# mlvlab/BLiM

Measured on AMD Instinct MI355X. Metric: candidate-pairs/sec (7B, 96+32 tok), higher is better.
Workload: dtype f16; 1 GPU; SYN v2t-VTG re-rank: Qwen2-7B dims (28 layers), seeded synthetic weights, 96 video + 32 text tokens per pair, top-16 text candidates per video query, 55 queries (880 pairs, 32560 packed tokens, 28160 label rows) per step per GPU; prefix_reuse=True, vtg_compensated=none, parallelism=query rows sharded over 1 GPU(s); RCCL all-gather of score rows at the end

## Files before the change

### blim_amd/csrc/gemm.hip

```cpp
#include "gemm.hpp"
#include "kernels.hpp"
#include <type_traits>

#define BM 256
#define BN 256
#define BK 64
#define NTHREADS 512
#define TILE_BYTES (BM * BK * 2)
#define BUF_BYTES (2 * TILE_BYTES)
#define GROUP_M 8

typedef const __attribute__((address_space(1))) void* gptr_t;
typedef __attribute__((address_space(3))) void* lptr_t;

__device__ __forceinline__ void glds16(const void* g, char* lds_wave_base) {
    __builtin_amdgcn_global_load_lds((gptr_t)g, (lptr_t)lds_wave_base, 16, 0, 0);
}

__device__ __forceinline__ float gelu_erf(float x) {
    const float z = fabsf(x) * 0.70710678118654752f;
    const float t = __builtin_amdgcn_rcpf(fmaf(0.3275911f, z, 1.0f));
    const float poly = t * fmaf(t, fmaf(t, fmaf(t, fmaf(t, 1.061405429f, -1.453152027f), 1.421413741f), -0.284496736f), 0.254829592f);
    const float erf_abs = 1.0f - poly * __expf(-z * z);
    return 0.5f * x * (1.0f + copysignf(erf_abs, x));
// ... 189 lines not shown
                    }
                    dma1(q);
                }
#ifdef GEMM_ABLATE_WREAD
#pragma unroll
                for (int ks = 0; ks < 2; ++ks)
#pragma unroll
                    for (int r = 0; r < 4; ++r) fb[ks][r] = fa[ks][r + 4];
#endif
            }
        };
        typedef int i32x2 __attribute__((ext_vector_type(2)));
        const char* g6A = LO6 ? (const char*)p.A6 + (int64_t)tm * nk6 * F6_TILE_BYTES : nullptr;
        const char* g6W = LO6 ? (const char*)p.W6 + (int64_t)tn * nk6 * F6_TILE_BYTES : nullptr;
        uint2 sc6a = make_uint2(0, 0);
        uint32_t sc6w = 0;
        auto dma6 = [&](int q, int dslot, int kd, bool isW, bool on) __attribute__((always_inline)) {
#if defined(GEMM_ABLATE_P2) && GEMM_ABLATE_P2 == 3
            on = on && kd < 3;
#endif
#if defined(GEMM_ABLATE_P2) && GEMM_ABLATE_P2 >= 4
            on = on && !((q == 4 || q == 5) && (isW || GEMM_ABLATE_P2 == 5));
#endif
            if (on) {
                const char* g = (isW ? g6W : g6A) + (int64_t)kd * F6_TILE_BYTES;
                char* d = smem + dslot * F6_TILE_BYTES;
                uint32_t o16 = (uint32_t)lane * 16u;
                asm volatile("" : "+v"(o16));
                if (q < 6) glds16(g + (wg + 4 * q) * 1024 + o16, d + (wg + 4 * q) * 1024);
                else if (lane < 16) glds16(g + 24576 + wg * 256 + o16, d + 24576 + wg * 256);
            }
        };
        auto stage6 = [&](int slot, int k, bool isW) __attribute__((always_inline)) {
#pragma unroll
            for (int q = 0; q < 7; ++q) dma6(q, slot, k, isW, true);
        };
        auto rd6 = [&](const char* qa, const char* qb, int off) __attribute__((always_inline)) {
            const i32x4 l = *(const i32x4*)(qa + off);
            const i32x2 h = *(const i32x2*)(qb + off);
            return (i32x8){l[0], l[1], l[2], l[3], h[0], h[1], 0, 0};
        };
#if defined(GEMM_ABLATE_P2) && GEMM_ABLATE_P2 >= 4
        auto rd6_4 = [&](const char* qa, const char* qb, int off) __attribute__((always_inline)) {
            const i32x4 l = *(const i32x4*)(qa + off);
            return (i32x8){l[0], l[1], l[2], l[3], l[0], l[1], 0, 0};
        };
#define RD6W rd6_4
#if GEMM_ABLATE_P2 == 5
#define RD6A rd6_4
#else
#define RD6A rd6
#endif
#else
#define RD6W rd6
#define RD6A rd6
#endif
        typedef int i32x1 __attribute__((ext_vector_type(1)));
        auto rd6_sw = [&](const char* tb) __attribute__((always_inline)) {
            return (uint32_t)(*(const i32x1*)(tb + 24576 + wn * 256 + lane * 4))[0];
        };
        auto rd6_sa = [&](const char* ta) __attribute__((always_inline)) {
            const i32x2 v = *(const i32x2*)(ta + 24576 + wm * 512 + lane * 8);
            return make_uint2((uint32_t)v[0], (uint32_t)v[1]);
        };
        int sa = 0;
        mx_request(0);
        if (grp == 0) {
            stage8(TILE_BYTES, 0);
            if (nk > 1) stage8(3 * TILE_BYTES, 1);
            if (nk > 1) asm volatile("s_waitcnt vmcnt(8)" ::: "memory");
            else asm volatile("s_waitcnt vmcnt(0)" ::: "memory");
            PHASE_BARRIER();
            if constexpr (MX8) mx_cur = mx_nxt;
            if constexpr (DT == DT_F8) {
                int sp = 0;
                for (int k = 0; k < nk; ++k) {
                    mx_request(k + 1);
                    load_frags(sa, adv(sa, 1));
                    if (k >= 1 && k + 1 < nk) stage8(sp, k + 1);
                    PHASE_BARRIER();
                    compute();
                    asm volatile("s_waitcnt vmcnt(0)" ::: "memory");
                    if constexpr (MX8) mx_cur = mx_nxt;
                    PHASE_BARRIER();
                    sp = sa; sa = adv(sa, 2);
                }
                PHASE_BARRIER();
            } else {
            load_frags(0, TILE_BYTES);
            PHASE_BARRIER();
            for (int kt = 0; kt < nk; ++kt) {
                WP_T(0);
                compute();
                WP_T(1);
                asm volatile("s_waitcnt vmcnt(0)" ::: "memory");
                WP_T(2);
                PHASE_BARRIER();
                WP_T(3);
                if constexpr (LO6) { if (kt + 1 == nk) break; }
                if (kt + 1 < nk) frags_and_dma(adv(sa, 2), adv(sa, 3), sa, kt + 2, kt + 2 < nk);
#ifdef GEMM_WAIT_PROF
                asm volatile("s_waitcnt lgkmcnt(0)" ::: "memory");
#endif
                WP_T(4);
                PHASE_BARRIER();
                WP_T(5);
                WP_ACC();
                sa = adv(sa, 2);
            }
            if constexpr (LO6) {
                stage6(0, 0, false); stage6(1, 0, true);
                if (nk6 > 1) { stage6(2, 1, false); stage6(3, 1, true); }
                if (nk6 > 2) { stage6(4, 2, false); stage6(5, 2, true); }
                PHASE_BARRIER();
            }
            }
        } else {
            stage8(0, 0);
            if (nk > 1) stage8(2 * TILE_BYTES, 1);
            if (nk > 1) asm volatile("s_waitcnt vmcnt(8)" ::: "memory");
            else asm volatile("s_waitcnt vmcnt(0)" ::: "memory");
            PHASE_BARRIER();
            if constexpr (MX8) mx_cur = mx_nxt;
            PHASE_BARRIER();
            for (int kt = 0; kt < nk; ++kt) {
                WP_T(0);
                if constexpr (DT == DT_F8) {
                    mx_request(kt + 1);
                    load_frags(sa, adv(sa, 1));
                    if (kt + 2 < nk) stage8(adv(sa, 4), kt + 2);
                } else frags_and_dma(sa, adv(sa, 1), adv(sa, 4), kt + 2, kt + 2 < nk);
#ifdef GEMM_WAIT_PROF
                asm volatile("s_waitcnt lgkmcnt(0)" ::: "memory");
#endif
                WP_T(1);
                if (kt + 2 < nk) asm volatile("s_waitcnt vmcnt(8)" ::: "memory");
                else asm volatile("s_waitcnt vmcnt(0)" ::: "memory");
                WP_T(2);
                PHASE_BARRIER();
                WP_T(3);
                compute();
                if constexpr (MX8) mx_cur = mx_nxt;
                WP_T(4);
                PHASE_BARRIER();
                WP_T(5);
                WP_ACC();
                sa = adv(sa, 2);
            }
        }
        if constexpr (LO6) {
#define P2_VMCNT(n) asm volatile("s_waitcnt vmcnt(" #n ")" ::: "memory")
#define P2_BARRIER() PHASE_BARRIER()
            if (grp == 0) {
                if (nk6 > 2) P2_VMCNT(28);
                else if (nk6 > 1) P2_VMCNT(14);
                else P2_VMCNT(0);
            }
            P2_BARRIER();
            const int qoa = 8 * wm * 1536 + lane * 16, qoa8 = 8 * wm * 1536 + 1024 + lane * 8;
            const int qob = F6_TILE_BYTES + 4 * wn * 1536 + lane * 16, qob8 = F6_TILE_BYTES + 4 * wn * 1536 + 1024 + lane * 8;
            sc6w = rd6_sw(smem + F6_TILE_BYTES); sc6a = rd6_sa(smem);
            fb8[0] = RD6W(smem + qob, smem + qob8, 0); fb8[1] = RD6W(smem + qob, smem + qob8, 1536);
#pragma unroll
            for (int i = 0; i < 4; ++i) fa8[i] = RD6A(smem + qoa, smem + qoa8, i * 1536);
            int s3 = 0;
#ifdef GEMM_WAIT_PROF
            for (int q_ = 0; q_ < 5; ++q_) wp_acc[q_] = 0;
#endif
#if defined(GEMM_ABLATE_P2) && GEMM_ABLATE_P2 == 1
#define L6_MMA(MI, NI)
#else
#define L6_MMA(MI, NI) acc[MI][NI] = __builtin_amdgcn_mfma_scale_f32_16x16x128_f8f6f4(fb8[NI], fa8[MI], acc[MI][NI], 2, 2, NI, (int)sc6w, (MI & 3), (int)((MI) < 4 ? sc6a.x : sc6a.y));
#endif
#define L6_SB() __builtin_amdgcn_sched_barrier(0)
            auto step6 = [&](int k, auto ca_, auto cb_) __attribute__((always_inline)) {
                constexpr int CA = decltype(ca_)::value, CB = decltype(cb_)::value;
                const int s3n = s3 == 2 ? 0 : s3 + 1, s3p = s3 == 0 ? 2 : s3 - 1;
                const char* t0 = smem + (2 * s3) * F6_TILE_BYTES;
                const char* t1 = smem + (2 * s3n) * F6_TILE_BYTES;
#if defined(GEMM_ABLATE_P2) && GEMM_ABLATE_P2 == 2
                const bool rl = false, own = false;
#else
                const bool rl = k + 1 < nk6, own = true;
#endif
                const bool on2 = k >= 1 && k + 2 < nk6;
                const bool on3 = k + 3 < nk6;
                const int d2 = 2 * s3p + (grp == 0 ? 1 : 0), d3 = 2 * s3 + (grp == 0 ? 1 : 0);
                const bool isW = grp == 0;
                uint2 sc6a_n = sc6a; uint32_t sc6w_n = sc6w;
                WP_T(0);
                __builtin_amdgcn_s_setprio(1);
                L6_MMA(0, CA) L6_SB(); if (own) fb8[CB] = RD6W(t0 + qob, t0 + qob8, CB * 1536); L6_SB();
                L6_MMA(1, CA) L6_SB(); dma6(4, d2, k + 2, isW, on2); L6_SB();
                L6_MMA(2, CA) L6_SB(); if (own) fb8[CB + 1] = RD6W(t0 + qob, t0 + qob8, (CB + 1) * 1536); L6_SB();
                L6_MMA(3, CA) L6_SB();
                L6_MMA(0, CA + 1) L6_SB(); if (own) fa8[4] = RD6A(t0 + qoa, t0 + qoa8, 4 * 1536); L6_SB();
                L6_MMA(1, CA + 1) L6_SB(); dma6(5, d2, k + 2, isW, on2); L6_SB();
                L6_MMA(2, CA + 1) L6_SB(); if (own) fa8[5] = RD6A(t0 + qoa, t0 + qoa8, 5 * 1536); L6_SB();
                L6_MMA(3, CA + 1) L6_SB();
                L6_MMA(0, CB) L6_SB(); if (own) fa8[6] = RD6A(t0 + qoa, t0 + qoa8, 6 * 1536); L6_SB();
                L6_MMA(1, CB) L6_SB(); if (own) fa8[7] = RD6A(t0 + qoa, t0 + qoa8, 7 * 1536); L6_SB();
                L6_MMA(2, CB) L6_SB(); dma6(6, d2, k + 2, isW, on2); L6_SB();
                L6_MMA(3, CB)
                L6_MMA(0, CB + 1) L6_MMA(1, CB + 1) L6_MMA(2, CB + 1) L6_MMA(3, CB + 1)
                L6_SB();
                WP_T(1);
#if defined(GEMM_ABLATE_P2) && GEMM_ABLATE_P2 == 6
                if (k == 0) { if (nk6 > 2) P2_VMCNT(21); else P2_VMCNT(0); }
                else if (k + 2 < nk6) P2_VMCNT(14);
                else P2_VMCNT(0);
#else
                if (k == 0) { if (nk6 > 2) P2_VMCNT(14); else P2_VMCNT(0); }
                else if (k + 2 < nk6) P2_VMCNT(7);
                else P2_VMCNT(0);
#endif
                WP_T(2);
#if defined(GEMM_ABLATE_P2) && GEMM_ABLATE_P2 == 7
                if (k & 1) { asm volatile("s_waitcnt lgkmcnt(0)" ::: "memory"); } else { P2_BARRIER(); }
#else
                P2_BARRIER();
#endif
                WP_T(3);
                L6_MMA(4, CB) L6_SB(); if (rl) fa8[0] = RD6A(t1 + qoa, t1 + qoa8, 0); L6_SB();
                L6_MMA(5, CB) L6_SB(); dma6(0, d3, k + 3, isW, on3); L6_SB();
                L6_MMA(6, CB) L6_SB(); if (rl) fa8[1] = RD6A(t1 + qoa, t1 + qoa8, 1536); L6_SB();
                L6_MMA(7, CB) L6_SB(); dma6(1, d3, k + 3, isW, on3); L6_SB();
                L6_MMA(4, CB + 1) L6_SB(); if (rl) { sc6w_n = rd6_sw(t1 + F6_TILE_BYTES); sc6a_n = rd6_sa(t1); } L6_SB();
                L6_MMA(5, CB + 1) L6_MMA(6, CB + 1) L6_MMA(7, CB + 1)
                L6_SB();
                WP_T(4);
                if (rl) fb8[CB] = RD6W(t1 + qob, t1 + qob8, CB * 1536);
                L6_SB();
                L6_MMA(4, CA) L6_SB(); if (rl) fb8[CB + 1] = RD6W(t1 + qob, t1 + qob8, (CB + 1) * 1536); L6_SB();
                L6_MMA(5, CA) L6_SB(); dma6(2, d3, k + 3, isW, on3); L6_SB();
                L6_MMA(6, CA) L6_SB(); if (rl) fa8[2] = RD6A(t1 + qoa, t1 + qoa8, 2 * 1536); L6_SB();
                L6_MMA(7, CA) L6_SB(); dma6(3, d3, k + 3, isW, on3); L6_SB();
                L6_MMA(4, CA + 1) L6_SB(); if (rl) fa8[3] = RD6A(t1 + qoa, t1 + qoa8, 3 * 1536); L6_SB();
                L6_MMA(5, CA + 1) L6_MMA(6, CA + 1) L6_MMA(7, CA + 1)
                L6_SB();
                __builtin_amdgcn_s_setprio(0);
                sc6a = sc6a_n; sc6w = sc6w_n;
                WP_T(5);
                WP_ACC();
                s3 = s3n;
            };
            {
                int k = 0;
                for (; k + 1 < nk6; k += 2) {
                    step6(k, std::integral_constant<int, 0>{}, std::integral_constant<int, 2>{});
                    step6(k + 1, std::integral_constant<int, 2>{}, std::integral_constant<int, 0>{});
                }
                if (k < nk6) step6(k, std::integral_constant<int, 0>{}, std::integral_constant<int, 2>{});
            }
#undef L6_SB
#undef RD6W
#undef RD6A
#undef P2_BARRIER
#undef P2_VMCNT
#undef L6_MMA
        }
#undef PHASE_BARRIER
#ifdef GEMM_WAIT_PROF
        if (p.debug_stamps && lane == 0 && (wave & 3) == 0)
            for (int q_ = 0; q_ < 5; ++q_) p.debug_stamps[((size_t)nwg + (size_t)stamp_vb * 2 + grp) * 8 + q_] = wp_acc[q_];
#endif
    }

    stamp(2);
    int tid_e = tid;
    asm volatile("" : "+v"(tid_e));
    if constexpr (out16<DT>::value == DT_F16) { if (p.f16_saturate) f16_saturate_on(); }
    else if constexpr (LO6_BF16_FENCE) { if (p.f16_saturate) f16_saturate_off(); }
    if (p.debug_skip_epilogue) {
#pragma unroll
        for (int i = 0; i < 8; ++i)
#pragma unroll
            for (int j = 0; j < 4; ++j) asm volatile("" ::"v"(acc[i][j]));
        __syncthreads();
        continue;
    }
    const int wrow0 = row0 + 128 * wm;
    const int wcol0 = col0 + 64 * wn;
    if constexpr (DT == DT_F8) {
        float* sc = (float*)smem;
        sc[tid_e] = f8_scale;
        __syncthreads();
        float4 cs[4];
#pragma unroll
        for (int ni = 0; ni < 4; ++ni) cs[ni] = *(const float4*)(sc + 256 + 64 * wn + 16 * ni + 4 * (lane >> 4));
#pragma unroll
        for (int mi = 0; mi < 8; ++mi) {
            const float rs = sc[128 * wm + 16 * mi + (lane & 15)];
#pragma unroll
            for (int ni = 0; ni < 4; ++ni) {
                acc[mi][ni][0] *= rs * cs[ni].x; acc[mi][ni][1] *= rs * cs[ni].y; acc[mi][ni][2] *= rs * cs[ni].z; acc[mi][ni][3] *= rs * cs[ni].w;
            }
        }
        __syncthreads();
    }

    if constexpr (EPI == EPI_LSE) {
        float2* red = (float2*)smem;
        const int q4 = lane >> 4;
#pragma unroll
        for (int mi = 0; mi < 8; ++mi) {
            const int rl = 128 * wm + 16 * mi + fr;
            const int row = row0 + rl;
            int lab = (row < p.M) ? p.labels[row] : -1;
            if (lab >= p.N) lab = -1;
            float v[4][4];
            float mx = -INFINITY;
#pragma unroll
            for (int ni = 0; ni < 4; ++ni)
#pragma unroll
                for (int j = 0; j < 4; ++j) {
                    const int col = wcol0 + 16 * ni + 4 * q4 + j;
                    v[ni][j] = (col < p.N) ? acc[mi][ni][j] : -INFINITY;
                    if (col == lab) p.label_logit[row] = v[ni][j];
                    mx = fmaxf(mx, v[ni][j]);
                }
            mx = fmaxf(mx, __shfl_xor(mx, 16)); mx = fmaxf(mx, __shfl_xor(mx, 32));
            float sm = 0.f;
            if (mx > -INFINITY) {
#pragma unroll
                for (int ni = 0; ni < 4; ++ni)
#pragma unroll
                    for (int j = 0; j < 4; ++j) sm += __expf(v[ni][j] - mx);
            }
            sm += __shfl_xor(sm, 16); sm += __shfl_xor(sm, 32);
            if (q4 == 0) red[wn * 256 + rl] = make_float2(mx, sm);
        }
        __syncthreads();
        if (tid_e < 256) {
            const int row = row0 + tid_e;
            if (row < p.M) {
                float2 a0 = red[tid_e], a1 = red[256 + tid_e], a2 = red[512 + tid_e], a3 = red[768 + tid_e];
                const float mx = fmaxf(fmaxf(a0.x, a1.x), fmaxf(a2.x, a3.x));
                float sm = 0.f;
                if (mx > -INFINITY) {
                    sm = a0.y * __expf(a0.x - mx) + a1.y * __expf(a1.x - mx) + a2.y * __expf(a2.x - mx) + a3.y * __expf(a3.x - mx);
                }
                p.lse_part[(int64_t)row * ntn + tn] = make_float2(mx, sm);
            }
        }
        stamp(3);
        __syncthreads();
        continue;
    } else {
        int tq = lane >> 4;
        int rsub = lane & 15;
        asm volatile("" : "+v"(tq), "+v"(rsub));
        __syncthreads();
        if constexpr (EPI == EPI_BF16 || EPI == EPI_QKV || EPI == EPI_SWIGLU) {
            constexpr int NC = (EPI == EPI_SWIGLU) ? 128 : 256;
            constexpr int RS = NC * 2 + 16;
            if constexpr (EPI == EPI_SWIGLU && DT == DT_F8) {
                if (p.out_mx != nullptr) {
                    float* red = (float*)smem;
                    uint8_t* st8 = (uint8_t*)smem + 8192;
                    constexpr int RS8 = 144;
#pragma unroll
                    for (int mi = 0; mi < 8; ++mi) {
                        float m = 0.f;
#pragma unroll
                        for (int pr = 0; pr < 2; ++pr)
#pragma unroll
                            for (int j = 0; j < 4; ++j) {
                                const float x = silu_f(acc[mi][2 * pr][j]) * acc[mi][2 * pr + 1][j];
                                acc[mi][2 * pr][j] = x;
                                m = fmaxf(m, fabsf(x));
                            }
                        m = fmaxf(m, __shfl_xor(m, 16)); m = fmaxf(m, __shfl_xor(m, 32));
                        if (tq == 0) red[wn * 256 + 128 * wm + 16 * mi + rsub] = m;
                    }
                    __syncthreads();
                    float* qinv = (float*)(smem + 4096);
                    if (tid_e < 256) {
                        const float a = fmaxf(fmaxf(red[tid_e], red[256 + tid_e]), fmaxf(red[512 + tid_e], red[768 + tid_e]));
                        int e = 0;
                        if (a > 0.f) {
                            int ex; const float mant = frexpf(a * (1.0f / FP8_MAX), &ex);
                            e = (mant == 0.5f) ? ex - 1 : ex;
                            if (ldexpf(a, -e) > FP8_MAX) e += 1;
                            e = max(-127, min(127, e));
                        }
                        qinv[tid_e] = ldexpf(1.0f, -e);
                        p.out_mx[(int64_t)tn * p.mx_stride + (int64_t)tm * 256 + ((tid_e >> 7) * 16 + (tid_e & 15)) * 8 + ((tid_e >> 4) & 7)] = (uint8_t)(e + 127);
                    }
                    __syncthreads();
#pragma unroll
                    for (int mi = 0; mi < 8; ++mi) {
                        const int rl = 128 * wm + 16 * mi + rsub;
                        const float inv = qinv[rl];
#pragma unroll
                        for (int pr = 0; pr < 2; ++pr)
                            *(uint32_t*)(st8 + rl * RS8 + (2 * wn + pr) * 16 + 4 * tq) =
                                pack_fp8x4(acc[mi][2 * pr][0] * inv, acc[mi][2 * pr][1] * inv, acc[mi][2 * pr][2] * inv, acc[mi][2 * pr][3] * inv);
                    }
                    __syncthreads();
                    const int64_t ob0 = col0 / 2;
#pragma unroll
                    for (int i = 0; i < 4; ++i) {
                        const int chunk = tid_e + NTHREADS * i, rl = chunk >> 3, seg = chunk & 7;
                        const int row = row0 + rl;
                        if (row < p.M && ob0 + seg * 16 + 15 < p.N / 2)
                            *(uint4*)((uint8_t*)p.C + (int64_t)row * p.ldc + ob0 + seg * 16) = *(const uint4*)(st8 + rl * RS8 + seg * 16);
                    }
                    stamp(3);
                    __syncthreads();
                    continue;
                }
            }
            constexpr int PROWS = SPLIT ? 128 : 256;
            constexpr int LO_OFF = PROWS * RS;
            static_assert(!SPLIT || 2 * LO_OFF <= 5 * TILE_BYTES, "hi + lo tiles of a half must fit the ring");
            auto ST = [&](char* o_, float a_, float b_, float c_, float d_) __attribute__((always_inline)) {
                const uint2 hi_ = make_uint2(pack2<ODT>(a_, b_), pack2<ODT>(c_, d_));
                *(uint2*)o_ = hi_;
                if constexpr (SPLIT) {
                    const uint16_t* h16_ = (const uint16_t*)&hi_;
                    *(uint2*)(o_ + LO_OFF) = make_uint2(pack2<ODT>(a_ - from16<ODT>(h16_[0]), b_ - from16<ODT>(h16_[1])), pack2<ODT>(c_ - from16<ODT>(h16_[2]), d_ - from16<ODT>(h16_[3])));
                }
            };
            constexpr int NMI = SPLIT ? 4 : 8;
#pragma unroll 1
            for (int hp = 0; hp < (SPLIT ? 2 : 1); ++hp) {
            const int mg0 = SPLIT ? 4 * hp : 0;
            const int lrow0 = SPLIT ? 64 * wm : 128 * wm;
            if (SPLIT && hp) {
                __syncthreads();
#pragma unroll
                for (int mi = 0; mi < 4; ++mi)
#pragma unroll
                    for (int ni = 0; ni < 4; ++ni) acc[mi][ni] = acc[(mi + 4) & 7][ni];
            }
            {
            float4 qkv_bias[4];
            if constexpr (EPI == EPI_QKV) {
#pragma unroll
                for (int ni = 0; ni < 4; ++ni) {
                    const int col = wcol0 + 16 * ni + 4 * tq;
                    qkv_bias[ni] = col + 3 < p.N ? *(const float4*)(p.bias + col) : make_float4(0.f, 0.f, 0.f, 0.f);
                }
            }
            float4 bf16_bias[4];
            if constexpr (EPI == EPI_BF16) {
#pragma unroll
                for (int ni = 0; ni < 4; ++ni) {
                    const int col = wcol0 + 16 * ni + 4 * tq;
                    bf16_bias[ni] = (p.bias && col + 3 < p.N) ? *(const float4*)(p.bias + col) : make_float4(0.f, 0.f, 0.f, 0.f);
                    if (p.bias && col < p.N && col + 3 >= p.N) {
                        bf16_bias[ni].x = p.bias[col];
                        if (col + 1 < p.N) bf16_bias[ni].y = p.bias[col + 1];
                        if (col + 2 < p.N) bf16_bias[ni].z = p.bias[col + 2];
                    }
                }
            }
            if constexpr (EPI == EPI_QKV) {
                if (wcol0 < p.rope_cols) {
                    const int hl = wn >> 1;
                    const int gbase = (wn & 1) * 2;
                    const int d0 = 16 * gbase + 4 * tq;
                    float4 cs[2][2], sn[2][2];
                    const int64_t cstride = p.rope_stride * 16;
                    auto request = [&](int mi, int buf) __attribute__((always_inline)) {
                        const int row = min(row0 + 128 * wm + 16 * (mg0 + mi) + rsub, p.M - 1);
                        const float* base = p.rope_rows + (int64_t)row * 16 + 4 * tq;
                        cs[buf][0] = *(const float4*)(base + (gbase + 0) * cstride); cs[buf][1] = *(const float4*)(base + (gbase + 1) * cstride);
                        sn[buf][0] = *(const float4*)(base + (4 + gbase + 0) * cstride); sn[buf][1] = *(const float4*)(base + (4 + gbase + 1) * cstride);
                    };
                    request(0, 0);
#pragma unroll
                    for (int mi = 0; mi < NMI; ++mi) {
                        if (mi + 1 < NMI) request(mi + 1, (mi + 1) & 1);
                        __builtin_amdgcn_sched_barrier(0);
                        char* lrow = smem + (lrow0 + 16 * mi + rsub) * RS;
#pragma unroll
                        for (int pr = 0; pr < 2; ++pr) {
                            const float4 c = cs[mi & 1][pr], sv = sn[mi & 1][pr];
                            const float c4[4] = {c.x, c.y, c.z, c.w}, s4[4] = {sv.x, sv.y, sv.z, sv.w};
                            const float4 b0 = qkv_bias[2 * pr], b1 = qkv_bias[2 * pr + 1];
                            const float bl[4] = {b0.x, b0.y, b0.z, b0.w}, bh[4] = {b1.x, b1.y, b1.z, b1.w};
                            float lo[4], hi[4];
#pragma unroll
                            for (int j = 0; j < 4; ++j) {
                                const float x1 = acc[mi][2 * pr][j] + bl[j];
                                const float x2 = acc[mi][2 * pr + 1][j] + bh[j];
                                lo[j] = x1 * c4[j] - x2 * s4[j];
                                hi[j] = x2 * c4[j] + x1 * s4[j];
                            }
                            char* o = lrow + (hl * 128 + d0 + 16 * pr) * 2;
                            ST(o, lo[0], lo[1], lo[2], lo[3]);
                            ST(o + 128, hi[0], hi[1], hi[2], hi[3]);
                        }
                    }
                } else {
#pragma unroll
                    for (int mi = 0; mi < NMI; ++mi) {
                        char* lrow = smem + (lrow0 + 16 * mi + rsub) * RS;
#pragma unroll
                        for (int ni = 0; ni < 4; ++ni) {
                            const float4 bv = qkv_bias[ni];
                            ST(lrow + (64 * wn + 16 * ni + 4 * tq) * 2, acc[mi][ni][0] + bv.x, acc[mi][ni][1] + bv.y, acc[mi][ni][2] + bv.z, acc[mi][ni][3] + bv.w);
                        }
                    }
                }
            } else
#pragma unroll
            for (int mi = 0; mi < NMI; ++mi) {
                const int rl = lrow0 + 16 * mi + rsub;
                float t[4][4];
#pragma unroll
                for (int ni = 0; ni < 4; ++ni) { t[ni][0] = acc[mi][ni][0]; t[ni][1] = acc[mi][ni][1]; t[ni][2] = acc[mi][ni][2]; t[ni][3] = acc[mi][ni][3]; }
                char* lrow = smem + rl * RS;
                if constexpr (EPI == EPI_BF16) {
                    if (p.bias == nullptr && p.act == 0) {
#pragma unroll
                        for (int ni = 0; ni < 4; ++ni)
                            ST(lrow + (64 * wn + 16 * ni + 4 * tq) * 2, t[ni][0], t[ni][1], t[ni][2], t[ni][3]);
                    } else if (p.act == 1) {
#pragma unroll
                        for (int ni = 0; ni < 4; ++ni) {
                            const float4 b = bf16_bias[ni];
                            ST(lrow + (64 * wn + 16 * ni + 4 * tq) * 2, gelu_erf(t[ni][0] + b.x), gelu_erf(t[ni][1] + b.y), gelu_erf(t[ni][2] + b.z), gelu_erf(t[ni][3] + b.w));
                        }
                    } else {
#pragma unroll
                        for (int ni = 0; ni < 4; ++ni) {
                            const float4 b = bf16_bias[ni];
                            ST(lrow + (64 * wn + 16 * ni + 4 * tq) * 2, t[ni][0] + b.x, t[ni][1] + b.y, t[ni][2] + b.z, t[ni][3] + b.w);
                        }
                    }
                } else {
#pragma unroll
                    for (int pr = 0; pr < 2; ++pr) {
                        const int cl = (2 * wn + pr) * 16 + 4 * tq;
                        float x[4];
#pragma unroll
                        for (int j = 0; j < 4; ++j) x[j] = silu_f(t[2 * pr][j]) * t[2 * pr + 1][j];
                        ST(lrow + cl * 2, x[0], x[1], x[2], x[3]);
                    }
                }
            }
            }
            __syncthreads();
            stamp(4);
            bool lo_as_tiles = false;
            if constexpr (EPI == EPI_SWIGLU && SPLIT && LO6) {
                if (p.out6 != nullptr) {
                    lo_as_tiles = true;
                    const int r = tid_e & 15, g = (tid_e >> 4) & 3, fl = tid_e >> 6;
                    const int ls = 64 * (fl >> 2) + 16 * (fl & 3) + r;
                    const int rl = 128 * (fl >> 2) + 64 * hp + 16 * (fl & 3) + r;
                    F6Block q;
                    if (row0 + rl < p.M) {
                        float f[32];
                        const char* src = smem + LO_OFF + ls * RS + g * 64;
#pragma unroll
                        for (int c4 = 0; c4 < 4; ++c4) {
                            const uint4 v = *(const uint4*)(src + 16 * c4);
                            const uint16_t* e16 = (const uint16_t*)&v;
#pragma unroll
                            for (int j = 0; j < 8; ++j) f[8 * c4 + j] = from16<ODT>(e16[j]);
                        }
                        q = e2m3_block(f);
                    } else { q.d[0] = q.d[1] = q.d[2] = q.d[3] = q.d[4] = q.d[5] = 0u; q.e8 = 0u; }
                    uint8_t* t = p.out6 + ((int64_t)tm * ntn + tn) * F6_TILE_BYTES;
                    const int fb = rl >> 4;
                    *(uint4*)(t + fb * 1536 + g * 256 + r * 16) = make_uint4(q.d[0], q.d[1], q.d[2], q.d[3]);
                    *(uint2*)(t + fb * 1536 + 1024 + g * 128 + r * 8) = make_uint2(q.d[4], q.d[5]);
                    t[24576 + ((rl >> 7) * 4 + g) * 128 + (rl & 15) * 8 + ((rl >> 4) & 7)] = (uint8_t)q.e8;
                }
            }
            constexpr int LPR = NC * 2 / 16;
            const int n_out = (EPI == EPI_SWIGLU) ? p.N / 2 : p.N;
            const int oc0 = (EPI == EPI_SWIGLU) ? col0 / 2 : col0;
            const int seg = tid_e % LPR;
            const int oc = oc0 + 8 * seg;
            constexpr int RPP = NTHREADS / LPR;
            bool fused_done = false;
            if constexpr (EPI == EPI_BF16 && !SPLIT) {
                if (p.swiglu_gu != nullptr) {
                    constexpr int ODT = out16<DT>::value;
                    int lds0 = (tid_e / LPR) * RS + seg * 16;
                    asm volatile("" : "+v"(lds0));
#pragma unroll 2
                    for (int rl = tid_e / LPR; rl < 256; rl += RPP) {
                        const int row = row0 + rl;
                        if (row >= p.M || oc >= n_out) continue;
                        const uint4 dv = *(const uint4*)(smem + lds0 + (rl - tid_e / LPR) * RS);
                        uint16_t* gp = p.swiglu_gu + (int64_t)row * p.swiglu_ld + 32 * (oc >> 4) + (oc & 15);
                        const uint4 gr = *(const uint4*)gp, ur = *(const uint4*)(gp + 16);
                        const uint16_t* dh = (const uint16_t*)&dv; const uint16_t* gh = (const uint16_t*)&gr; const uint16_t* uh = (const uint16_t*)&ur;
                        uint4 og, ou;
                        uint16_t* pg = (uint16_t*)&og; uint16_t* pu = (uint16_t*)&ou;
#pragma unroll
                        for (int e = 0; e < 8; ++e) {
                            const float g = from16<ODT>(gh[e]), u = from16<ODT>(uh[e]), d = from16<ODT>(dh[e]);
                            const float sg = __builtin_amdgcn_rcpf(1.0f + __expf(-g));
                            pg[e] = to16<ODT>(d * u * sg * (1.0f + g * (1.0f - sg)));
                            pu[e] = to16<ODT>(d * g * sg);
                        }
                        *(uint4*)gp = og;
                        *(uint4*)(gp + 16) = ou;
                    }
                    fused_done = true;
                }
            }
            auto tile_row = [&](int rl_) __attribute__((always_inline)) { return SPLIT ? 128 * (rl_ >> 6) + 64 * hp + (rl_ & 63) : rl_; };
            if (fused_done) {
            } else if (row0 + 256 <= p.M && oc0 + NC <= n_out && (p.ldc & 7) == 0) {
                constexpr int NV = PROWS / RPP;
                uint4 v[NV];
                static_assert(64 % RPP == 0, "a thread's rows i * RPP must not straddle a 64-row staging block");
                const char* lsrc = smem + (tid_e / LPR) * RS + seg * 16;
                bf16_t* out = (bf16_t*)p.C + (int64_t)(row0 + tid_e / LPR) * p.ldc + oc;
#pragma unroll
                for (int i = 0; i < NV; ++i) v[i] = *(const uint4*)(lsrc + i * RPP * RS);
#pragma unroll
                for (int i = 0; i < NV; ++i) *(uint4*)(out + (int64_t)tile_row(i * RPP) * p.ldc) = v[i];
                if (SPLIT && !lo_as_tiles) {
                    __builtin_amdgcn_sched_barrier(0);
#pragma unroll
                    for (int i = 0; i < NV; ++i) v[i] = *(const uint4*)(lsrc + LO_OFF + i * RPP * RS);
#pragma unroll
                    for (int i = 0; i < NV; ++i) *(uint4*)(out + p.lo_off + (int64_t)tile_row(i * RPP) * p.ldc) = v[i];
                }
                if constexpr (EPI == EPI_BF16 && !SPLIT) {
                    if (p.swiglu_act != nullptr && (seg & 3) < 2) {
                        constexpr int ODT = out16<DT>::value;
                        uint16_t* aout = p.swiglu_act + (int64_t)(row0 + tid_e / LPR) * p.swiglu_act_ld + oc0 / 2 + 16 * (seg >> 2) + 8 * (seg & 3);
#pragma unroll
                        for (int i = 0; i < 256 / RPP; ++i) {
                            const uint4 ur = *(const uint4*)(lsrc + i * RPP * RS + 32);
                            const uint16_t* gh = (const uint16_t*)&v[i]; const uint16_t* uh = (const uint16_t*)&ur;
                            uint4 o; uint16_t* po = (uint16_t*)&o;
#pragma unroll
                            for (int e = 0; e < 8; ++e) { const float g = from16<ODT>(gh[e]); po[e] = to16<ODT>(silu_f(g) * from16<ODT>(uh[e])); }
                            *(uint4*)(aout + (int64_t)i * RPP * p.swiglu_act_ld) = o;
                        }
                    }
                }
            } else
#pragma unroll 1
            for (int rl = tid_e / LPR; rl < PROWS; rl += RPP) {
                const int row = row0 + tile_row(rl);
                if (row >= p.M || oc >= n_out) continue;
                const uint4 v = *(const uint4*)(smem + rl * RS + seg * 16);
                bf16_t* out = (bf16_t*)p.C + (int64_t)row * p.ldc + oc;
                auto store8 = [&](bf16_t* o_, const uint4 v_) __attribute__((always_inline)) {
                    if (oc + 7 < n_out && (p.ldc & 7) == 0) *(uint4*)o_ = v_;
                    else {
                        const uint32_t w_[4] = {v_.x, v_.y, v_.z, v_.w};
#pragma unroll
                        for (int j = 0; j < 8; ++j)
                            if (oc + j < n_out) o_[j] = (bf16_t)(w_[j >> 1] >> (16 * (j & 1)));
                    }
                };
                store8(out, v);
                if (SPLIT && !lo_as_tiles) store8(out + p.lo_off, *(const uint4*)(smem + LO_OFF + rl * RS + seg * 16));
                if constexpr (EPI == EPI_BF16 && !SPLIT) {
                    if (p.swiglu_act != nullptr && (seg & 3) < 2) {
                        constexpr int ODT = out16<DT>::value;
                        const uint4 ur = *(const uint4*)(smem + rl * RS + seg * 16 + 32);
                        const uint16_t* gh = (const uint16_t*)&v; const uint16_t* uh = (const uint16_t*)&ur;
                        uint4 o; uint16_t* po = (uint16_t*)&o;
#pragma unroll
                        for (int e = 0; e < 8; ++e) { const float g = from16<ODT>(gh[e]); po[e] = to16<ODT>(silu_f(g) * from16<ODT>(uh[e])); }
                        *(uint4*)(p.swiglu_act + (int64_t)row * p.swiglu_act_ld + oc0 / 2 + 16 * (seg >> 2) + 8 * (seg & 3)) = o;
                    }
                }
            }
            stamp(5);
            }
        } else {
            constexpr int RS = 1024 + 16;
#pragma unroll 1
            for (int h = 0; h < 2; ++h) {
                if (wm == h) {
#pragma unroll
                    for (int mi = 0; mi < 8; ++mi) {
                        char* lrow = smem + (16 * mi + rsub) * RS;
#pragma unroll
                        for (int ni = 0; ni < 4; ++ni) {
                            *(float4*)(lrow + (64 * wn + 16 * ni + 4 * tq) * 4) = make_float4(acc[mi][ni][0], acc[mi][ni][1], acc[mi][ni][2], acc[mi][ni][3]);
                        }
                    }
                }
                __syncthreads();
                const int col = col0 + 4 * lane;
                const bool vec = (col + 3 < p.N) && ((p.ldc & 3) == 0);
                if constexpr (EPI == EPI_RESID) {
                    const float* rsrc = p.resid_in ? p.resid_in : (const float*)p.C;
                    if (vec) {
                        const float4 rb = p.bias ? *(const float4*)(p.bias + col) : make_float4(0.f, 0.f, 0.f, 0.f);
                        float4 o[16];
#pragma unroll
                        for (int i = 0; i < 16; ++i) {
                            const int row = min(row0 + 128 * h + wave + 8 * i, p.M - 1);
                            o[i] = *(const float4*)(rsrc + (int64_t)row * p.ldc + col);
                        }
#pragma unroll
                        for (int i = 0; i < 16; ++i) {
                            const int rl = wave + 8 * i;
                            const int row = row0 + 128 * h + rl;
                            const float4 v = *(const float4*)(smem + rl * RS + lane * 16);
                            if (row < p.M) *(float4*)((float*)p.C + (int64_t)row * p.ldc + col) = make_float4(o[i].x + (v.x + rb.x), o[i].y + (v.y + rb.y), o[i].z + (v.z + rb.z), o[i].w + (v.w + rb.w));
#ifdef GEMM_ABLATE_NORMFOLD
                            if (p.swiglu_act != nullptr && row < p.M) {
                                const float4 nv = make_float4(o[i].x + (v.x + rb.x), o[i].y + (v.y + rb.y), o[i].z + (v.z + rb.z), o[i].w + (v.w + rb.w));
                                float ss = nv.x * nv.x + nv.y * nv.y + nv.z * nv.z + nv.w * nv.w;
#pragma unroll
                                for (int m_ = 1; m_ < 64; m_ <<= 1) ss += __shfl_xor(ss, m_);
                                const float r = rsqrtf(ss * (1.0f / 256.0f) + 1e-6f);
                                const float4 wv = *(const float4*)(p.col_scale + col);
                                const uint16_t h0 = to16<ODT>(nv.x * wv.x * r), h1 = to16<ODT>(nv.y * wv.y * r), h2 = to16<ODT>(nv.z * wv.z * r), h3 = to16<ODT>(nv.w * wv.w * r);
                                *(uint2*)(p.swiglu_act + (int64_t)row * p.swiglu_act_ld + col) = make_uint2((uint32_t)h0 | ((uint32_t)h1 << 16), (uint32_t)h2 | ((uint32_t)h3 << 16));
                                if (lane == 0) ((float*)p.lse_part)[(int64_t)row * ntn + tn] = ss;
                            }
#endif
                        }
                    } else {
#pragma unroll 1
                        for (int i = 0; i < 16; ++i) {
                            const int rl = wave + 8 * i;
                            const int row = row0 + 128 * h + rl;
                            if (row >= p.M || col >= p.N) continue;
                            const float4 v = *(const float4*)(smem + rl * RS + lane * 16);
                            const float x[4] = {v.x, v.y, v.z, v.w};
                            float* out = (float*)p.C + (int64_t)row * p.ldc + col;
                            const float* in = rsrc + (int64_t)row * p.ldc + col;
#pragma unroll
                            for (int j = 0; j < 4; ++j)
                                if (col + j < p.N) out[j] = in[j] + x[j] + (p.bias ? p.bias[col + j] : 0.f);
                        }
                    }
                } else {
#pragma unroll 4
                    for (int i = 0; i < 16; ++i) {
                        const int rl = wave + 8 * i;
                        const int row = row0 + 128 * h + rl;
                        if (row >= p.M || col >= p.N) continue;
                        const float4 v = *(const float4*)(smem + rl * RS + lane * 16);
                        float x[4] = {v.x * p.scale, v.y * p.scale, v.z * p.scale, v.w * p.scale};
                        float* out = (float*)p.C + (int64_t)row * p.ldc + col;
                        if (vec) *(float4*)out = make_float4(x[0], x[1], x[2], x[3]);
                        else {
#pragma unroll
                            for (int j = 0; j < 4; ++j)
                                if (col + j < p.N) out[j] = x[j];
                        }
                    }
                }
                __syncthreads();
            }
        }
        if (p.debug_stamps) asm volatile("s_waitcnt vmcnt(0)" ::: "memory");
        stamp(3);
        __syncthreads();
    }
    }
}

#define NBM 64
#define NBN 64
#define NRING 4
#define N_A_BYTES (NBM * 128)
#define N_STEP_BYTES ((NBM + NBN) * 128)
#define N_THREADS 256
__device__ __forceinline__ void narrow_resid_epilogue(const GemmParams& p, const f32x4 (&acc)[2][2], int wrow0, int wcol0, int lane) {
    const int tq = lane >> 4, rsub = lane & 15;
    const float* rsrc = p.resid_in ? p.resid_in : (const float*)p.C;
#pragma unroll
    for (int mi = 0; mi < 2; ++mi) {
        const int row = wrow0 + 16 * mi + rsub;
#pragma unroll
        for (int ni = 0; ni < 2; ++ni) {
            const int col = wcol0 + 16 * ni + 4 * tq;
            if (row >= p.M || col >= p.N) continue;
            const f32x4 v = acc[mi][ni];
            float* out = (float*)p.C + (int64_t)row * p.ldc + col;
            const float* in = rsrc + (int64_t)row * p.ldc + col;
            if ((col + 3 < p.N) && ((p.ldc & 3) == 0)) {
                const float4 rb = p.bias ? *(const float4*)(p.bias + col) : make_float4(0.f, 0.f, 0.f, 0.f);
                const float4 o = *(const float4*)in;
                *(float4*)out = make_float4(o.x + (v[0] + rb.x), o.y + (v[1] + rb.y), o.z + (v[2] + rb.z), o.w + (v[3] + rb.w));
            } else {
                const float x[4] = {v[0], v[1], v[2], v[3]};
#pragma unroll
                for (int j = 0; j < 4; ++j)
                    if (col + j < p.N) out[j] = in[j] + x[j] + (p.bias ? p.bias[col + j] : 0.f);
            }
        }
    }
}
__device__ __forceinline__ void narrow_tile(const GemmParams& p, int bid, int& tm, int& tn) {
    const int ntm = (p.M + NBM - 1) / NBM, ntn = (p.N + NBN - 1) / NBN;
    const int nwg = ntm * ntn;
    const int xcd = bid & 7, cq = nwg >> 3, cr = nwg & 7;
    const int pid = (xcd < cr ? xcd * (cq + 1) : cr * (cq + 1) + (xcd - cr) * cq) + (bid >> 3);
    const int width = p.group_m * ntn;
    const int first_m = (pid / width) * p.group_m;
    const int gsz = min(ntm - first_m, p.group_m);
    tm = first_m + (pid % width) % gsz;
    tn = (pid % width) / gsz;
}
template <int DT>
__global__ __launch_bounds__(N_THREADS) void gemm_narrow_kernel(const GemmParams p) {
    __shared__ __attribute__((aligned(16))) char smem[NRING * N_STEP_BYTES];
    const int tid = threadIdx.x;
    const int lane = tid & 63;
    const int wave = __builtin_amdgcn_readfirstlane(tid >> 6);
    const int wm = wave >> 1, wn = wave & 1;
    int tm, tn;
    narrow_tile(p, blockIdx.x, tm, tn);
    const int row0 = tm * NBM, col0 = tn * NBN;

    const int sr = lane >> 3;
    const int sc = (lane & 7) ^ (4 * (wave & 1) + (sr >> 1));
    const int64_t w_ld = p.w_wrap_k > 0 ? p.w_wrap_k : p.K;
    uint32_t offA[2], offW[2];
#pragma unroll
    for (int i = 0; i < 2; ++i) {
        const int b = wave + 4 * i;
        offA[i] = (uint32_t)((int64_t)min(row0 + 8 * b + sr, p.M - 1) * p.lda * 2 + 16 * sc);
        offW[i] = (uint32_t)((int64_t)min(col0 + 8 * b + sr, p.N - 1) * w_ld * 2 + 16 * sc);
    }
    const char* baseA = (const char*)p.A;
    const char* baseW = (const char*)p.W;
    const int nk = p.K / 64;
    const int wrap = p.w_wrap_k > 0 ? p.w_wrap_k / 64 : 0x7fffffff;
    auto stage = [&](int slot, int kt) __attribute__((always_inline)) {
        const char* ga = baseA + (int64_t)kt * 128;
        const char* gw = baseW + (int64_t)(kt >= wrap ? kt - wrap : kt) * 128;
        char* d = smem + slot * N_STEP_BYTES + wave * 1024;
#pragma unroll
        for (int i = 0; i < 2; ++i) {
            uint32_t oa = offA[i], ow = offW[i];
            asm volatile("" : "+v"(oa), "+v"(ow));
            glds16(ga + oa, d + i * 4096);
            glds16(gw + ow, d + N_A_BYTES + i * 4096);
        }
    };
// ... 619 lines not shown
```

Measured before the change: 2626 pairs/s.

## Restructure LSE epilogue and software-pipeline SwiGLU epilogue transcendentals

The LSE epilogue now loads labels up front, specialises the max/sum sweep for interior tiles so column bounds checks drop out, and picks the label logit with a single owning-lane select after the sweep instead of comparing inside the inner loop. The SwiGLU epilogue is rewritten as a manually software-pipelined sequence of packed exp2/rcp/mul stages with scheduling barriers, so transcendental latency overlaps across elements. This adds code complexity and register pressure from the staged arrays, and fixes the instruction order, which limits what the compiler's scheduler can do.

```diff
diff --git a/blim_amd/csrc/gemm.hip b/blim_amd/csrc/gemm.hip
--- a/blim_amd/csrc/gemm.hip
+++ b/blim_amd/csrc/gemm.hip
@@ -515,33 +515,60 @@
     if constexpr (EPI == EPI_LSE) {
         float2* red = (float2*)smem;
         const int q4 = lane >> 4;
+        int labs[8];
+        int lrow_e = 128 * wm + fr;
+        asm volatile("" : "+v"(lrow_e));
+#pragma unroll
+        for (int mi = 0; mi < 8; ++mi) labs[mi] = p.labels[min(row0 + lrow_e + 16 * mi, p.M - 1)];
+        float2 part[8];
+        auto sweep = [&](auto interior_) __attribute__((always_inline)) {
+            constexpr bool INTERIOR = decltype(interior_)::value;
+#pragma unroll
+            for (int mi = 0; mi < 8; ++mi) {
+                float v[4][4];
+                float mx = -INFINITY;
+#pragma unroll
+                for (int ni = 0; ni < 4; ++ni)
+#pragma unroll
+                    for (int j = 0; j < 4; ++j) {
+                        const int col = wcol0 + 16 * ni + 4 * q4 + j;
+                        v[ni][j] = (INTERIOR || col < p.N) ? acc[mi][ni][j] : -INFINITY;
+                        mx = fmaxf(mx, v[ni][j]);
+                    }
+                mx = fmaxf(mx, __shfl_xor(mx, 16)); mx = fmaxf(mx, __shfl_xor(mx, 32));
+                float sm = 0.f;
+                if (mx > -INFINITY) {
+#pragma unroll
+                    for (int ni = 0; ni < 4; ++ni)
+#pragma unroll
+                        for (int j = 0; j < 4; ++j) sm += __expf(v[ni][j] - mx);
+                }
+                sm += __shfl_xor(sm, 16); sm += __shfl_xor(sm, 32);
+                part[mi] = make_float2(mx, sm);
+            }
+        };
+        if (col0 + 256 <= p.N) sweep(std::true_type{});
+        else sweep(std::false_type{});
+        if (q4 == 0) {
+#pragma unroll
+            for (int mi = 0; mi < 8; ++mi) red[wn * 256 + lrow_e + 16 * mi] = part[mi];
+        }
 #pragma unroll
         for (int mi = 0; mi < 8; ++mi) {
-            const int rl = 128 * wm + 16 * mi + fr;
-            const int row = row0 + rl;
-            int lab = (row < p.M) ? p.labels[row] : -1;
+            const int row = row0 + lrow_e + 16 * mi;
+            int lab = (row < p.M) ? labs[mi] : -1;
             if (lab >= p.N) lab = -1;
-            float v[4][4];
-            float mx = -INFINITY;
-#pragma unroll
-            for (int ni = 0; ni < 4; ++ni)
-#pragma unroll
-                for (int j = 0; j < 4; ++j) {
-                    const int col = wcol0 + 16 * ni + 4 * q4 + j;
-                    v[ni][j] = (col < p.N) ? acc[mi][ni][j] : -INFINITY;
-                    if (col == lab) p.label_logit[row] = v[ni][j];
-                    mx = fmaxf(mx, v[ni][j]);
-                }
-            mx = fmaxf(mx, __shfl_xor(mx, 16)); mx = fmaxf(mx, __shfl_xor(mx, 32));
-            float sm = 0.f;
-            if (mx > -INFINITY) {
+            const unsigned loff = (unsigned)lab - (unsigned)wcol0;
+            if (loff < 64u && ((loff >> 2) & 3u) == (unsigned)q4) {
+                const unsigned sel = loff & ~12u;
+                float pick = acc[mi][0][0];
 #pragma unroll
                 for (int ni = 0; ni < 4; ++ni)
 #pragma unroll
-                    for (int j = 0; j < 4; ++j) sm += __expf(v[ni][j] - mx);
-            }
-            sm += __shfl_xor(sm, 16); sm += __shfl_xor(sm, 32);
-            if (q4 == 0) red[wn * 256 + rl] = make_float2(mx, sm);
+                    for (int j = 0; j < 4; ++j)
+                        if (sel == (unsigned)(16 * ni + j)) pick = acc[mi][ni][j];
+                p.label_logit[row] = pick;
+            }
         }
         __syncthreads();
         if (tid_e < 256) {
@@ -718,6 +745,35 @@
                         }
                     }
                 }
+            } else if constexpr (EPI == EPI_SWIGLU) {
+                typedef float f2 __attribute__((ext_vector_type(2)));
+                constexpr int NP = 4 * NMI;
+                const f2 nl2e = {-1.44269504088896340736f, -1.44269504088896340736f};
+                char* l0 = smem + (lrow0 + rsub) * RS + (32 * wn + 4 * tq) * 2;
+                f2 m[NP], e[NP], d[NP], r[NP], s[NP], x[NP];
+#define SW_G(n) f2{acc[(n) >> 2][2 * (((n) >> 1) & 1)][2 * ((n) & 1)], acc[(n) >> 2][2 * (((n) >> 1) & 1)][2 * ((n) & 1) + 1]}
+#define SW_U(n) f2{acc[(n) >> 2][2 * (((n) >> 1) & 1) + 1][2 * ((n) & 1)], acc[(n) >> 2][2 * (((n) >> 1) & 1) + 1][2 * ((n) & 1) + 1]}
+#define SW_IN(n) ((n) >= 0 && (n) < NP)
+                m[0] = SW_G(0) * nl2e;
+#pragma unroll
+                for (int i = 0; i < NP + 5; ++i) {
+                    if (SW_IN(i)) e[i].x = __builtin_amdgcn_exp2f(m[i].x);
+                    if (SW_IN(i + 1)) m[i + 1] = SW_G(i + 1) * nl2e;
+                    if (SW_IN(i)) e[i].y = __builtin_amdgcn_exp2f(m[i].y);
+                    if (SW_IN(i - 1)) d[i - 1] = 1.0f + e[i - 1];
+                    if (SW_IN(i - 2)) r[i - 2].x = __builtin_amdgcn_rcpf(d[i - 2].x);
+                    if (SW_IN(i - 3)) s[i - 3] = SW_G(i - 3) * r[i - 3];
+                    if (SW_IN(i - 2)) r[i - 2].y = __builtin_amdgcn_rcpf(d[i - 2].y);
+                    if (SW_IN(i - 4)) x[i - 4] = s[i - 4] * SW_U(i - 4);
+                    if (SW_IN(i - 5) && ((i - 5) & 1)) {
+                        const int n = i - 5;
+                        ST(l0 + (n >> 2) * 16 * RS + ((n >> 1) & 1) * 32, x[n - 1].x, x[n - 1].y, x[n].x, x[n].y);
+                    }
+                    __builtin_amdgcn_sched_barrier(0);
+                }
+#undef SW_IN
+#undef SW_U
+#undef SW_G
             } else
 #pragma unroll
             for (int mi = 0; mi < NMI; ++mi) {
@@ -743,15 +799,6 @@
                             const float4 b = bf16_bias[ni];
                             ST(lrow + (64 * wn + 16 * ni + 4 * tq) * 2, t[ni][0] + b.x, t[ni][1] + b.y, t[ni][2] + b.z, t[ni][3] + b.w);
                         }
-                    }
-                } else {
-#pragma unroll
-                    for (int pr = 0; pr < 2; ++pr) {
-                        const int cl = (2 * wn + pr) * 16 + 4 * tq;
-                        float x[4];
-#pragma unroll
-                        for (int j = 0; j < 4; ++j) x[j] = silu_f(t[2 * pr][j]) * t[2 * pr + 1][j];
-                        ST(lrow + cl * 2, x[0], x[1], x[2], x[3]);
                     }
                 }
             }
```

Result: no change. 2637 pairs/s, median of 6 (+0.4%).
